# julienperriercornet/turbosqueeze

Measured on AMD Instinct MI355X. Metric: encode+decode GB/s on enwik9-shaped input (round trip of uncompressed bytes), higher is better.
Workload: dtype u8

## Files before the change

### include/turbosqueeze_amd.h

```cpp
#ifndef TURBOSQUEEZE_AMD_H
#define TURBOSQUEEZE_AMD_H

#include <stdbool.h>
#include <stddef.h>
#include <stdint.h>
#include <stdio.h>

#ifdef __cplusplus
extern "C" {
#endif

#ifndef TSQ_BLOCK_BITS
#define TSQ_BLOCK_BITS (22)
#define TSQ_BLOCK_SZ   (1 << TSQ_BLOCK_BITS)
#define TSQ_OUTPUT_SZ  ((1 << TSQ_BLOCK_BITS) + (1 << (TSQ_BLOCK_BITS - 2)))
#define TSQ_HASH_BITS  (17)
#define TSQ_HASH_SZ    ((1 << TSQ_HASH_BITS) * sizeof(uint16_t))
#define TSQ_HASH_MASK  ((1 << TSQ_HASH_BITS) - 1)
#endif

enum {
    TSQA_OK            = 0,
    TSQA_ERR_NO_DEVICE = 1,
    TSQA_ERR_HIP       = 2,
// ... 45 lines not shown
    uint32_t pad;
} tsqa_frame;

int tsqa_decode_blocks_async(tsqa_ctx *ctx, const void *d_streams, const tsqa_frame *d_frames, uint32_t n_blocks,
                             void *d_out, int32_t *d_status, void *hip_stream);

int tsqa_frames_to_host_async(tsqa_ctx *ctx, const void *d_slots, const uint32_t *sizes, const uint64_t *frame_at,
                              uint32_t n_blocks, uint32_t ext, void *host_container, void *hip_stream);
int tsqa_frames_from_host_async(tsqa_ctx *ctx, const void *host_container, const uint64_t *frame_at, const uint32_t *sizes,
                                uint32_t n_blocks, void *d_streams, void *hip_stream);

int tsqa_profile_enable(tsqa_ctx *ctx, int on);
int tsqa_profile_read(tsqa_ctx *ctx, double *encode_ms, uint32_t *encode_launches,
                      double *decode_ms, uint32_t *decode_launches);
int tsqa_profile_read_calls(tsqa_ctx *ctx, double *compress_ms, uint32_t *compress_calls,
                            double *decompress_ms, uint32_t *decompress_calls);

int tsqa_frame_offsets(const uint32_t *sizes, uint32_t n_blocks, uint64_t *frame_at, uint64_t *container_size);
int tsqa_walk_frames(const void *container, size_t size, uint32_t cap_blocks, uint64_t *frame_at, uint32_t *sizes, uint32_t *ext,
                     uint32_t *out_len, uint32_t *n_blocks, uint64_t *total);
int tsqa_sharded_place_async(tsqa_ctx *ctx, const void *d_slots, const uint32_t *all_sizes, uint32_t n_blocks, uint64_t n_total,
                             uint32_t rank, uint32_t world, uint32_t ext, void *host_container, size_t host_cap,
                             uint64_t *container_size, void *hip_stream);
int tsqa_sharded_fetch_decode_async(tsqa_ctx *ctx, const void *host_container, size_t container_size, uint32_t rank, uint32_t world,
                                    void *d_streams, size_t streams_cap, void *d_out, size_t out_cap, int32_t *d_status, uint64_t *total,
                                    void *hip_stream);
int tsqa_sharded_decode_again_async(tsqa_ctx *ctx, const void *d_streams, void *d_out, int32_t *d_status, void *hip_stream);

int tsqa_measure_copy(tsqa_ctx *ctx, size_t bytes, int reps, double *best_gbps, double *median_gbps);
const char *tsqa_copy_probe_shape(const tsqa_ctx *ctx);

void tsqa_set_kernel_variant(tsqa_ctx *ctx, int encode_variant, int decode_variant);
void tsqa_set_decode_wait_limit(tsqa_ctx *ctx, uint32_t polls);

typedef struct tsqa_index tsqa_index;
int      tsqa_index_create(tsqa_ctx *ctx, const void *d_container, size_t n, tsqa_index **out);
void     tsqa_index_destroy(tsqa_index *idx);
uint32_t tsqa_index_blocks(const tsqa_index *idx);
uint64_t tsqa_index_total(const tsqa_index *idx);

typedef struct tsqa_range { uint64_t offset, length, out_at; } tsqa_range;
typedef struct tsqa_range_item { uint32_t block, lo, hi, pad; uint64_t out_at; } tsqa_range_item;

int tsqa_plan_ranges(const uint64_t *out_start, uint32_t n_blocks, const tsqa_range *ranges, uint32_t n_ranges,
                     size_t out_cap, tsqa_range_item *items, uint32_t cap_items, uint32_t *n_items);

int tsqa_decompress_ranges_async(tsqa_ctx *ctx, const tsqa_index *idx, const tsqa_range *ranges, uint32_t n_ranges,
                                 void *d_out, size_t out_cap, int32_t *d_status, void *hip_stream);
int tsqa_decompress_ranges(tsqa_ctx *ctx, const tsqa_index *idx, const tsqa_range *ranges, uint32_t n_ranges,
                           void *d_out, size_t out_cap, void *hip_stream);

typedef struct tsqa_batch_item { uint64_t in_at, in_len, out_at, out_cap; } tsqa_batch_item;

int tsqa_plan_batch(const tsqa_batch_item *items, uint32_t n_items, size_t in_size, size_t out_size,
                    const uint32_t *n_blocks, uint64_t *first_block);

int tsqa_compress_batch_async(tsqa_ctx *ctx, const void *d_in, size_t in_size, const tsqa_batch_item *items, uint32_t n_items,
                              uint32_t ext, void *d_out, size_t out_size, uint64_t *d_sizes, int32_t *d_status, void *hip_stream);
int tsqa_compress_batch(tsqa_ctx *ctx, const void *d_in, size_t in_size, const tsqa_batch_item *items, uint32_t n_items,
                        uint32_t ext, void *d_out, size_t out_size, uint64_t *sizes, void *hip_stream);

int tsqa_decompress_batch_async(tsqa_ctx *ctx, const void *d_in, size_t in_size, const tsqa_batch_item *items,
                                const uint32_t *n_blocks, uint32_t n_items, void *d_out, size_t out_size,
                                uint64_t *d_sizes, int32_t *d_status, void *hip_stream);
int tsqa_decompress_batch(tsqa_ctx *ctx, const void *d_in, size_t in_size, const tsqa_batch_item *items, uint32_t n_items,
                          void *d_out, size_t out_size, uint64_t *sizes, int32_t *item_status, void *hip_stream);
// ... 121 lines not shown
```

### turbosqueeze_amd/api.py

```python
from __future__ import annotations

import ctypes as C
import os
import subprocess

HERE = os.path.dirname(os.path.abspath(__file__))
BLOCK_SZ = 1 << 22
OUTPUT_SZ = BLOCK_SZ + (BLOCK_SZ >> 2)

ERRORS = {1: "no usable gfx950 device", 2: "HIP runtime error", 3: "bad argument", 4: "malformed container",
          5: "malformed block stream", 6: "block expanded beyond TSQ_OUTPUT_SZ",
          7: "multi-workgroup decode stalled waiting for a sibling workgroup (the container may be fine: decode again with variant 4)"}


class TsqError(RuntimeError):
    def __init__(self, code: int, detail: str = ""):
        self.code = code
        super().__init__(f"turbosqueeze_amd error {code} ({ERRORS.get(code, '?')}) {detail}".strip())


def lib_path(ab=False) -> str:
    if isinstance(ab, str):
        return os.path.join(HERE, f"libturbosqueeze_amd_{ab}.so")
    return os.path.join(HERE, "libturbosqueeze_amd_ab.so" if ab else "libturbosqueeze_amd.so")
# ... 35 lines not shown
                          "(hipcc --offload-arch=gfx950); turbosqueeze_amd has no CPU fallback")
    L = C.CDLL(path)
    vp, u8pp, szp = C.c_void_p, C.POINTER(C.c_void_p), C.POINTER(C.c_size_t)
    L.tsqa_create.restype = C.c_int
    L.tsqa_create.argtypes = [C.c_int, C.POINTER(vp)]
    L.tsqa_destroy.restype = None
    L.tsqa_destroy.argtypes = [vp]
    L.tsqa_last_error.restype = C.c_char_p
    L.tsqa_last_error.argtypes = [vp]
    L.tsqa_device_id.restype = C.c_int
    L.tsqa_device_id.argtypes = [vp]
    L.tsqa_block_count.restype = C.c_size_t
    L.tsqa_block_count.argtypes = [C.c_size_t]
    L.tsqa_build_info.restype = C.c_char_p
    L.tsqa_build_info.argtypes = []
    L.tsqa_container_bound.restype = C.c_size_t
    L.tsqa_container_bound.argtypes = [C.c_size_t]
    L.tsqa_compress_device.restype = C.c_int
    L.tsqa_compress_device.argtypes = [vp, vp, C.c_size_t, vp, C.c_size_t, szp, C.c_uint32, vp]
    L.tsqa_compress_device_async.restype = C.c_int
    L.tsqa_compress_device_async.argtypes = [vp, vp, C.c_size_t, vp, C.c_size_t, vp, vp, C.c_uint32, vp]
    L.tsqa_decompress_device.restype = C.c_int
    L.tsqa_decompress_device.argtypes = [vp, vp, C.c_size_t, vp, C.c_size_t, szp, vp]
    L.tsqa_decompress_device_async.restype = C.c_int
    L.tsqa_decompress_device_async.argtypes = [vp, vp, C.c_size_t, C.c_uint32, vp, C.c_size_t, vp, vp, vp]
    L.tsqa_profile_enable.restype = C.c_int
    L.tsqa_profile_enable.argtypes = [vp, C.c_int]
    L.tsqa_profile_read.restype = C.c_int
    L.tsqa_profile_read.argtypes = [vp, C.POINTER(C.c_double), C.POINTER(C.c_uint32), C.POINTER(C.c_double), C.POINTER(C.c_uint32)]
    L.tsqa_set_kernel_variant.restype = None
    L.tsqa_set_kernel_variant.argtypes = [vp, C.c_int, C.c_int]
    L.tsqa_set_decode_wait_limit.restype = None
    L.tsqa_set_decode_wait_limit.argtypes = [vp, C.c_uint32]
    L.tsqAllocateContext.restype = vp
    L.tsqDeallocateContext.argtypes = [vp]
    L.tsqInit.argtypes = [vp]
    L.tsqEncode.restype = None
    L.tsqEncode.argtypes = [vp, vp, vp, C.POINTER(C.c_uint32), C.c_uint32, C.c_uint32]
    L.tsqDecode.restype = None
    L.tsqDecode.argtypes = [vp, vp, C.POINTER(C.c_uint32), C.c_uint32, C.c_uint32]
    L.tsqAllocateContextCompression_MT.restype = vp
    L.tsqAllocateContextCompression_MT.argtypes = [C.c_bool]
    L.tsqDeallocateContextCompression_MT.argtypes = [vp]
    L.tsqAllocateContextDecompression_MT.restype = vp
    L.tsqAllocateContextDecompression_MT.argtypes = [C.c_bool]
    L.tsqDeallocateContextDecompression_MT.argtypes = [vp]
    L.tsqCompress_MT.restype = C.c_bool
    L.tsqCompress_MT.argtypes = [vp, vp, C.c_size_t, C.c_bool, u8pp, szp, C.c_bool, C.c_bool, C.c_uint32]
    L.tsqDecompress_MT.restype = C.c_bool
    L.tsqDecompress_MT.argtypes = [vp, vp, C.c_size_t, C.c_bool, u8pp, szp, C.c_bool]
    L.tsqa_compress_async_cb.restype = C.c_uint32
    L.tsqa_compress_async_cb.argtypes = [vp, vp, C.c_size_t, C.c_bool, u8pp, szp, C.c_bool, C.c_bool, C.c_uint32, vp, vp, vp]
    L.tsqa_decompress_async_cb.restype = C.c_uint32
    L.tsqa_decompress_async_cb.argtypes = [vp, vp, C.c_size_t, C.c_bool, u8pp, szp, C.c_bool, vp, vp, vp]
    L.tsqa_profile_read_calls.restype = C.c_int
    L.tsqa_profile_read_calls.argtypes = [vp, C.POINTER(C.c_double), C.POINTER(C.c_uint32), C.POINTER(C.c_double), C.POINTER(C.c_uint32)]
    L.tsqa_encode_blocks_async.restype = C.c_int
    L.tsqa_encode_blocks_async.argtypes = [vp, vp, C.c_uint32, C.c_size_t, C.c_uint32, C.c_uint32, vp, vp, vp, vp]
    L.tsqa_decode_blocks_async.restype = C.c_int
    L.tsqa_decode_blocks_async.argtypes = [vp, vp, vp, C.c_uint32, vp, vp, vp]
    L.tsqa_frames_to_host_async.restype = C.c_int
    L.tsqa_frames_to_host_async.argtypes = [vp, vp, vp, vp, C.c_uint32, C.c_uint32, vp, vp]
    L.tsqa_frames_from_host_async.restype = C.c_int
    L.tsqa_frames_from_host_async.argtypes = [vp, vp, vp, vp, C.c_uint32, vp, vp]
    u32p, u64p = C.POINTER(C.c_uint32), C.POINTER(C.c_uint64)
    L.tsqa_frame_offsets.restype = C.c_int
# ... 457 lines not shown
        self.h = C.c_void_p()
        if device < 0:
            device = torch.cuda.current_device()
        rc = self.L.tsqa_create(device, C.byref(self.h))
        if rc:
            raise TsqError(rc)
        self.device = torch.device("cuda", device)
        self._size = torch.zeros(1, dtype=torch.int64, device=self.device)
        self._status = torch.zeros(1, dtype=torch.int32, device=self.device)

    def close(self):
        if self.h:
            self.L.tsqa_destroy(self.h)
            self.h = C.c_void_p()

    def __del__(self):
        try:
            self.close()
        except Exception:
            pass

    def _err(self, rc):
        return TsqError(rc, self.L.tsqa_last_error(self.h).decode())

    def last_error(self) -> str:
        return self.L.tsqa_last_error(self.h).decode()

    def set_variant(self, enc: int, dec: int) -> None:
        self.L.tsqa_set_kernel_variant(self.h, enc, dec)

    def set_decode_wait_limit(self, polls: int) -> None:
        self.L.tsqa_set_decode_wait_limit(self.h, polls)

    def profile(self, on: bool) -> None:
        self.L.tsqa_profile_enable(self.h, 1 if on else 0)

    def profile_read(self):
        em, dm, en, dn = C.c_double(0), C.c_double(0), C.c_uint32(0), C.c_uint32(0)
        self.L.tsqa_profile_read(self.h, C.byref(em), C.byref(en), C.byref(dm), C.byref(dn))
        return em.value, en.value, dm.value, dn.value

    def profile_read_calls(self):
        em, dm, en, dn = C.c_double(0), C.c_double(0), C.c_uint32(0), C.c_uint32(0)
        self.L.tsqa_profile_read_calls(self.h, C.byref(em), C.byref(en), C.byref(dm), C.byref(dn))
        return em.value, en.value, dm.value, dn.value

    def measure_copy(self, nbytes: int = 1 << 30, reps: int = 7):
        best, med = C.c_double(0), C.c_double(0)
        rc = self.L.tsqa_measure_copy(self.h, nbytes, reps, C.byref(best), C.byref(med))
        if rc:
            raise self._err(rc)
        return best.value, med.value

    def copy_probe_shape(self) -> str:
        return self.L.tsqa_copy_probe_shape(self.h).decode()

    def _stream(self):
        return C.c_void_p(self.torch.cuda.current_stream(self.device).cuda_stream)

    def encode_blocks_async(self, d_in, n_blocks: int, stride: int, last_len: int, ext: int, d_slots, d_sizes):
        rc = self.L.tsqa_encode_blocks_async(self.h, d_in.data_ptr(), n_blocks, stride, last_len, int(ext), d_slots.data_ptr(),
                                             d_sizes.data_ptr(), self._status.data_ptr(), self._stream())
        if rc:
            raise self._err(rc)

    def decode_blocks_async(self, d_streams, d_frames, n_blocks: int, d_out):
# ... 433 lines not shown
```

### turbosqueeze_amd/csrc/tsq_container.cuh

```cuda
#pragma once

#include "tsq_common.cuh"
#include "tsq_format.h"

namespace tsq {

__device__ __forceinline__ uint64_t group_scan_excl64(uint64_t v, uint64_t* wave_sum , uint64_t* total)
{
    const uint32_t lane = threadIdx.x & 63u, wid = threadIdx.x >> 6;
    const uint64_t incl = ((uint64_t)wave_scan_add((uint32_t)(v >> 24)) << 24) + wave_scan_add((uint32_t)v & 0xFFFFFFu);
    __syncthreads();
    if (lane == 63u) wave_sum[wid] = incl;
    __syncthreads();
    uint64_t before = 0, all = 0;
    for (uint32_t w = 0; w < 4u; ++w) { const uint64_t s = wave_sum[w]; if (w < wid) before += s; all += s; }
    *total = all;
    return before + incl - v;
}

__global__ __launch_bounds__(256) void pack_scan_kernel(const uint32_t* __restrict__ sizes, uint32_t n_blocks,
                                                        uint64_t n_total, uint32_t ext, uint8_t* __restrict__ container,
                                                        uint64_t out_cap, uint64_t* __restrict__ frame_at,
                                                        uint64_t* __restrict__ out_size, int32_t* __restrict__ status)
{
// ... 19 lines not shown

constexpr uint32_t kPackPiece = 32768;
__device__ __forceinline__ void pack_copy_piece(const uint8_t* src, uint32_t size, uint8_t* dst, uint32_t piece_at)
{
    const uint32_t head = (uint32_t)((16u - ((uintptr_t)dst & 15u)) & 15u);
    const uint32_t begin = piece_at + head;
    const uint32_t end_all = size;
    uint32_t end = begin + kPackPiece;
    if (end > end_all) end = end_all;
    if (piece_at == 0) for (uint32_t k = threadIdx.x; k < head && k < size; k += 256) dst[k] = src[k];
    if (begin >= end_all) return;
    const uint32_t words = (end - begin) >> 4;
    for (uint32_t w = threadIdx.x; w < words; w += 256) {
        uint4 v;
        __builtin_memcpy(&v, src + begin + (w << 4), 16);
        *reinterpret_cast<uint4*>(dst + begin + (w << 4)) = v;
    }
    if (end == end_all) for (uint32_t k = begin + (words << 4) + threadIdx.x; k < end_all; k += 256) dst[k] = src[k];
}

__global__ __launch_bounds__(256) void pack_copy_kernel(const uint8_t* __restrict__ slots, const uint32_t* __restrict__ sizes,
                                                        const uint64_t* __restrict__ frame_at, uint8_t* __restrict__ container,
                                                        const int32_t* __restrict__ status)
{
    const uint32_t b = blockIdx.y;
    const uint32_t size = sizes[b];
    const uint32_t piece_at = blockIdx.x * kPackPiece;
    if (piece_at >= size || *status != 0) return;
    pack_copy_piece(slots + (size_t)b * kSlotSize, size, container + frame_at[b] + 3, piece_at);
}

__global__ __launch_bounds__(64) void frame_walk_kernel(const uint8_t* __restrict__ container, uint64_t n, uint32_t n_blocks,
                                                        uint64_t out_cap, FrameInfo* __restrict__ frames,
                                                        uint64_t* __restrict__ out_size, int32_t* __restrict__ status)
{
    if (threadIdx.x != 0) return;
    uint32_t nb = 0;
    uint64_t total = 0;
    const bool ok = read_header(container, n, &nb, &total) == kHeaderOk && nb == n_blocks && total <= out_cap &&
                    walk_frames(container, n, nb, total, [&](uint32_t b, uint64_t, const FrameInfo& f) { frames[b] = f; return true; }) == kWalkOk;
    *out_size = ok ? total : 0;
    if (!ok) atomicMax(status, kErrFormat);
}

}
```

### turbosqueeze_amd/csrc/tsq_internal.h

```cpp
#pragma once

#include <hip/hip_runtime.h>
#include <stddef.h>
#include <stdint.h>
#include <utility>
#include <vector>

#include "../../include/turbosqueeze_amd.h"

namespace tsq { struct FrameInfo; struct BatchItem; struct EncBatchBlock; }

struct tsqa_ctx;

template <class T> struct tsqa_scratch {
    T* p = nullptr;
    size_t cap = 0;
    tsqa_scratch() = default;
    tsqa_scratch(const tsqa_scratch&) = delete;
    tsqa_scratch& operator=(const tsqa_scratch&) = delete;
    ~tsqa_scratch() { reset(); }
    operator T*() const { return p; }
    bool needs(size_t n) const { return n > cap; }
    void reset() { (void)hipFree(p); p = nullptr; cap = 0; }
    bool grow(tsqa_ctx* c, size_t n);
// ... 27 lines not shown

struct tsqa_ctx {
    int device = 0;
    int n_cus = 0;
    hipStream_t stream = nullptr;
    tsqa_scratch<uint8_t> slots;
    tsqa_scratch<uint32_t> sizes;
    tsqa_scratch<uint64_t> frame_at;
    tsqa_scratch<tsq::FrameInfo> frames;
    tsqa_scratch<uint32_t> block_owner;
    tsqa_scratch<uint16_t> tables;
    tsq::FrameInfo* host_frames = nullptr;
    size_t cap_host_frames = 0;
    std::vector<uint64_t> host_frame_src;
    hipEvent_t host_frames_copied = nullptr;
    bool host_frames_pending = false;
    uint32_t sharded_n_local = 0;
    const void* sharded_streams = nullptr;
    void* sharded_out = nullptr;
    void forget_sharded() { sharded_n_local = 0; sharded_streams = nullptr; sharded_out = nullptr; }
    tsqa_uploads range_up, batch_up;
    tsqa_scratch<int32_t> batch_status;
    tsqa_scratch<uint64_t> batch_at, batch_sizes, batch_offsets;
    tsqa_scratch<uint8_t> batch_heads;
    tsqa_scratch<tsq::BatchItem> batch_items;
    tsqa_scratch<uint32_t> batch_live;
    tsqa_scratch<tsq::EncBatchBlock> table_blocks;
    tsqa_scratch<uint32_t> table_launch_item;
    char probe_shape[160] = {0};
    tsqa_scratch<uint32_t> duo_ring;
    tsqa_scratch<uint32_t> duo_flags;
    tsqa_scratch<uint64_t> d_size;
    tsqa_scratch<int32_t> d_status;
    int enc_variant = 0, dec_variant = 0;
    uint32_t decode_wait_limit = 1u << 24;
    char err[256] = {0};
    static constexpr int kProfKinds = 4, kProfPairs = 256;
    bool profiling = false;
    std::vector<hipEvent_t> prof_pool;
    uint32_t prof_used[kProfKinds] = {0, 0, 0, 0};

    void set_error(const char* fmt, ...) __attribute__((format(printf, 2, 3)));
    void wait_for(hipStream_t s) { (void)hipStreamSynchronize(stream); if (s && s != stream) (void)hipStreamSynchronize(s); }
    int reserve(size_t n_blocks, bool want_tables, bool want_slots = true, bool all_streams = false, hipStream_t s = nullptr);
    int reserve_duo(size_t n_blocks, hipStream_t s = nullptr);
    int reserve_host_frames(size_t n);
    int reserve_batch(size_t n_items);
    int reserve_tables(size_t n_blocks, size_t n_launches);
    int launch_encode(const void* d_in, size_t n, size_t readable, uint32_t ext, int32_t* status, hipStream_t s);
    int launch_encode_to(const void* d_in, size_t n, size_t readable, size_t stride, uint32_t ext, uint8_t* slots_out,
                         uint32_t* sizes_out, int32_t* status, hipStream_t s);
    int launch_decode_frames(const void* d_streams, const tsq::FrameInfo* d_frames, uint32_t n_blocks, void* d_out, int32_t* status, hipStream_t s, int variant = -1);
    int decode_again(const void* d_streams, const tsq::FrameInfo* d_frames, uint32_t n_blocks, void* d_out, int32_t* status, hipStream_t s);
    int launch_pack(size_t n, uint32_t ext, void* d_out, size_t out_cap, uint64_t* d_out_size, int32_t* status, hipStream_t s);
};

template <class T> bool tsqa_scratch<T>::grow(tsqa_ctx* c, size_t n)
{
    if (!needs(n)) return true;
    reset();
    const hipError_t e = hipMalloc(&p, n * sizeof(T));
    if (e != hipSuccess) { p = nullptr; c->set_error("hipMalloc of %zu B failed: %s", n * sizeof(T), hipGetErrorString(e)); return false; }
    cap = n;
    return true;
}

// ... 15 lines not shown
```

### turbosqueeze_amd/csrc/tsq_runtime.hip

```cpp
#include "tsq_internal.h"

#include "tsq_batch.cuh"
#include "tsq_common.cuh"
#include "tsq_container.cuh"
#include "tsq_format.h"
#include "tsq_serial.cuh"
#include "tsq_split.cuh"
#include "tsq_index.cuh"
#include "tsq_launch.cuh"

#include <algorithm>
#include <cstdarg>
#include <cstdio>
#include <cstring>
#include <memory>
#include <new>

using namespace tsq;

#define TSQ_HIP(ctx, call)                                                                       \
    do {                                                                                         \
        hipError_t e_ = (call);                                                                  \
        if (e_ != hipSuccess) {                                                                  \
            (ctx)->set_error("%s failed: %s", #call, hipGetErrorString(e_));                     \
// ... 61 lines not shown
#endif
#ifdef TSQ_JITTER
           " TSQ_JITTER"
#endif
#if !TSQ_TIMING_ONLY_BUILD && !TSQ_INSTRUMENTED_BUILD
           " none"
#endif
           "]";
}

extern "C" int tsqa_create(int device, tsqa_ctx** out)
{
    if (!out) return TSQA_ERR_ARG;
    *out = nullptr;
    int count = 0;
    if (hipGetDeviceCount(&count) != hipSuccess || count <= 0) return TSQA_ERR_NO_DEVICE;
    if (device < 0) { if (hipGetDevice(&device) != hipSuccess) return TSQA_ERR_NO_DEVICE; }
    if (device >= count) return TSQA_ERR_ARG;
    hipDeviceProp_t prop;
    if (hipGetDeviceProperties(&prop, device) != hipSuccess) return TSQA_ERR_NO_DEVICE;
    if (strncmp(prop.gcnArchName, "gfx950", 6) != 0) {
        fprintf(stderr, "turbosqueeze_amd: device %d is %s; this library carries gfx950 code only\n", device, prop.gcnArchName);
        return TSQA_ERR_NO_DEVICE;
    }
    tsqa_ctx* c = new (std::nothrow) tsqa_ctx();
    if (!c) return TSQA_ERR_ARG;
    c->device = device;
    c->n_cus = prop.multiProcessorCount;
    if (const char* e = getenv("TSQ_AMD_DECODE_WAIT_LIMIT")) { const long v = atol(e); if (v > 0) c->decode_wait_limit = (uint32_t)v; }
    if (hipSetDevice(device) != hipSuccess || hipStreamCreateWithFlags(&c->stream, hipStreamNonBlocking) != hipSuccess) {
        delete c;
        return TSQA_ERR_HIP;
    }
    if (!c->d_size.grow(c, 1) || !c->d_status.grow(c, 1)) {
        tsqa_destroy(c);
        return TSQA_ERR_HIP;
    }
    *out = c;
    return TSQA_OK;
}

extern "C" void tsqa_destroy(tsqa_ctx* c)
{
    if (!c) return;
    (void)hipSetDevice(c->device);
    if (c->stream) { (void)hipStreamSynchronize(c->stream); (void)hipStreamDestroy(c->stream); }
    for (hipEvent_t e : c->prof_pool) if (e) (void)hipEventDestroy(e);
    if (c->host_frames) (void)hipHostFree(c->host_frames);
    if (c->host_frames_copied) (void)hipEventDestroy(c->host_frames_copied);
    c->range_up.destroy(); c->batch_up.destroy();
    delete c;
}

extern "C" const char* tsqa_last_error(const tsqa_ctx* c) { return c ? c->err : "null context"; }
extern "C" int tsqa_device_id(const tsqa_ctx* c) { return c ? c->device : -1; }
extern "C" void tsqa_set_kernel_variant(tsqa_ctx* c, int ev, int dv) { if (c) { c->enc_variant = ev; c->dec_variant = dv; } }
extern "C" void tsqa_set_decode_wait_limit(tsqa_ctx* c, uint32_t polls) { if (c) c->decode_wait_limit = polls ? polls : 1u; }

int tsqa_ctx::reserve(size_t n_blocks, bool want_tables, bool want_slots, bool all_streams, hipStream_t s)
{
    (void)hipSetDevice(device);
    const size_t nb = n_blocks, n_at = nb ? nb + 1 : 0;
    const size_t n_slots = want_slots && nb ? nb * (size_t)kSlotSize + 256 : 0, n_tables = want_tables ? nb * (size_t)kHashEntries : 0;
    const bool descriptors = sizes.needs(nb) || frame_at.needs(n_at) || frames.needs(nb) || block_owner.needs(nb);
    if (!descriptors && !slots.needs(n_slots) && !tables.needs(n_tables)) return TSQA_OK;
    if (all_streams) (void)hipDeviceSynchronize(); else wait_for(s);
    if (descriptors) forget_sharded();
    return sizes.grow(this, nb) && frame_at.grow(this, n_at) && frames.grow(this, nb) && block_owner.grow(this, nb) &&
           slots.grow(this, n_slots) && tables.grow(this, n_tables) ? TSQA_OK : TSQA_ERR_HIP;
}

int tsqa_ctx::reserve_duo(size_t n_blocks, hipStream_t s)
{
    (void)hipSetDevice(device);
    const size_t n_ring = n_blocks * (size_t)DuoCfg::SLOTS * DuoCfg::REC_WORDS, n_flags = n_blocks * (size_t)DuoCfg::FLAG_STRIDE;
    if (!duo_ring.needs(n_ring) && !duo_flags.needs(n_flags)) return TSQA_OK;
    wait_for(s);
    return duo_ring.grow(this, n_ring) && duo_flags.grow(this, n_flags) ? TSQA_OK : TSQA_ERR_HIP;
}

static size_t doubled(size_t from, size_t n)
{
    if (n == 0) return 0;
    while (from < n) from *= 2;
    return from;
}

int tsqa_ctx::reserve_host_frames(size_t n)
{
    (void)hipSetDevice(device);
    if (host_frames_pending) { (void)hipEventSynchronize(host_frames_copied); host_frames_pending = false; }
    if (!host_frames_copied) TSQ_HIP(this, hipEventCreateWithFlags(&host_frames_copied, hipEventDisableTiming));
    if (n > cap_host_frames) {
        if (host_frames) (void)hipHostFree(host_frames);
        host_frames = nullptr; cap_host_frames = 0;
        const size_t want = doubled(64, n);
        TSQ_HIP(this, hipHostMalloc(reinterpret_cast<void**>(&host_frames), want * sizeof(FrameInfo), hipHostMallocDefault));
        cap_host_frames = want;
    }
    host_frame_src.resize(cap_host_frames);
// ... 93 lines not shown
    }
    c->prof_used[kind] = 0;
    if (ms) *ms = sum;
    if (count) *count = n;
}

extern "C" int tsqa_profile_read(tsqa_ctx* c, double* enc_ms, uint32_t* enc_n, double* dec_ms, uint32_t* dec_n)
{
    if (!c) return TSQA_ERR_ARG;
    (void)hipSetDevice(c->device);
    if (c->prof_pool.empty()) { if (enc_ms) *enc_ms = 0; if (enc_n) *enc_n = 0; if (dec_ms) *dec_ms = 0; if (dec_n) *dec_n = 0; return TSQA_OK; }
    drain_events(c, 0, enc_ms, enc_n);
    drain_events(c, 1, dec_ms, dec_n);
    return TSQA_OK;
}

extern "C" int tsqa_profile_read_calls(tsqa_ctx* c, double* comp_ms, uint32_t* comp_n, double* decomp_ms, uint32_t* decomp_n)
{
    if (!c) return TSQA_ERR_ARG;
    (void)hipSetDevice(c->device);
    if (c->prof_pool.empty()) { if (comp_ms) *comp_ms = 0; if (comp_n) *comp_n = 0; if (decomp_ms) *decomp_ms = 0; if (decomp_n) *decomp_n = 0; return TSQA_OK; }
    drain_events(c, 2, comp_ms, comp_n);
    drain_events(c, 3, decomp_ms, decomp_n);
    return TSQA_OK;
}


int tsqa_ctx::launch_encode_to(const void* d_in, size_t n, size_t readable, size_t stride, uint32_t ext, uint8_t* slots_out,
                               uint32_t* sizes_out, int32_t* status, hipStream_t s)
{
    const uint32_t nb = (uint32_t)tsqa_block_count(n);
    int rc = reserve(nb, true, false, false, s);
    if (rc) return rc;
    ProfSpan span(this, 0, s);
    rc = launch_encode_kernels(this, static_cast<const uint8_t*>(d_in), n, readable, stride, ext, slots_out, sizes_out, status, s);
    if (rc) { span.cancel(); return rc; }
    span.end();
    TSQ_HIP(this, hipGetLastError());
    return TSQA_OK;
}

int tsqa_ctx::launch_encode(const void* d_in, size_t n, size_t readable, uint32_t ext, int32_t* status, hipStream_t s)
{
    int rc = reserve((uint32_t)tsqa_block_count(n), true, true, false, s);
    if (rc) return rc;
    return launch_encode_to(d_in, n, readable, kBlockSize, ext, slots, sizes, status, s);
}


static uint32_t pack_pieces(uint32_t max_stream = kSlotSize) { return (max_stream + kPackPiece - 1) / kPackPiece + 1; }

int tsqa_ctx::launch_pack(size_t n, uint32_t ext, void* d_out, size_t out_cap, uint64_t* d_out_size, int32_t* status, hipStream_t s)
{
    const uint32_t nb = (uint32_t)tsqa_block_count(n);
    hipLaunchKernelGGL(pack_scan_kernel, dim3(1), dim3(256), 0, s, sizes, nb, (uint64_t)n, ext,
                       static_cast<uint8_t*>(d_out), (uint64_t)out_cap, frame_at, d_out_size, status);
    hipLaunchKernelGGL(pack_copy_kernel, dim3(pack_pieces(), nb), dim3(256), 0, s, slots, sizes, frame_at,
                       static_cast<uint8_t*>(d_out), status);
    TSQ_HIP(this, hipGetLastError());
    return TSQA_OK;
}

int tsqa_ctx::launch_decode_frames(const void* d_streams, const FrameInfo* d_frames, uint32_t n_blocks, void* d_out, int32_t* status, hipStream_t s, int variant)
{
    ProfSpan span(this, 1, s);
    int rc = launch_decode_kernels(this, static_cast<const uint8_t*>(d_streams), d_frames, n_blocks, static_cast<uint8_t*>(d_out), status, s, variant);
    if (rc) { span.cancel(); return rc; }
    span.end();
    TSQ_HIP(this, hipGetLastError());
    return TSQA_OK;
}

int tsqa_ctx::decode_again(const void* d_streams, const FrameInfo* d_frames, uint32_t n_blocks, void* d_out, int32_t* status, hipStream_t s)
{
    TSQ_HIP(this, hipMemsetAsync(status, 0, sizeof(int32_t), s));
    return launch_decode_frames(d_streams, d_frames, n_blocks, d_out, status, s, 4);
}


extern "C" int tsqa_compress_device_async(tsqa_ctx* c, const void* d_in, size_t n, void* d_out, size_t out_cap,
                                          uint64_t* d_out_size, int32_t* d_status, uint32_t ext, void* hip_stream)
{
    if (!c) return TSQA_ERR_ARG;
    if (!d_in || !d_out || !d_out_size || !d_status || n == 0) { c->set_error("compress: null pointer or zero size"); return TSQA_ERR_ARG; }
    if (out_cap < 16 + 6 * tsqa_block_count(n)) { c->set_error("compress: output capacity too small"); return TSQA_ERR_ARG; }
    hipStream_t s = stream_of(c, hip_stream);
    (void)hipSetDevice(c->device);
    TSQ_HIP(c, hipMemsetAsync(d_status, 0, sizeof(int32_t), s));
    ProfSpan span(c, 2, s);
    int rc = c->launch_encode(d_in, n, n, ext, d_status, s);
    if (rc) { span.cancel(); return rc; }
    rc = c->launch_pack(n, ext, d_out, out_cap, d_out_size, d_status, s);
    span.end();
    return rc;
}

static int status_to_rc(tsqa_ctx* c, int32_t st, const char* what)
{
    if (st == 0) return TSQA_OK;
    c->set_error("%s: device reported status %d", what, st);
    return st;
}

static int read_status(tsqa_ctx* c, hipStream_t s, int32_t* st, size_t* out_size = nullptr)
{
    uint64_t sz = 0;
    if (out_size) TSQ_HIP(c, hipMemcpyAsync(&sz, c->d_size, sizeof(sz), hipMemcpyDeviceToHost, s));
    TSQ_HIP(c, hipMemcpyAsync(st, c->d_status, sizeof(int32_t), hipMemcpyDeviceToHost, s));
    TSQ_HIP(c, hipStreamSynchronize(s));
    if (out_size) *out_size = (size_t)sz;
    return TSQA_OK;
}
static int finish_sync(tsqa_ctx* c, hipStream_t s, const char* what, size_t* out_size = nullptr)
{
    int32_t st = 0;
    if (int rc = read_status(c, s, &st, out_size)) return rc;
    return status_to_rc(c, st, what);
}

extern "C" int tsqa_compress_device(tsqa_ctx* c, const void* d_in, size_t n, void* d_out, size_t out_cap,
                                    size_t* out_size, uint32_t ext, void* hip_stream)
{
    if (!c || !out_size) return TSQA_ERR_ARG;
    hipStream_t s = stream_of(c, hip_stream);
    int rc = tsqa_compress_device_async(c, d_in, n, d_out, out_cap, c->d_size, c->d_status, ext, s);
    if (rc) return rc;
    return finish_sync(c, s, "compress", out_size);
}

static int decompress_device_async_impl(tsqa_ctx* c, const void* d_in, size_t n, uint32_t n_blocks, void* d_out,
                                        size_t out_cap, uint64_t* d_out_size, int32_t* d_status, void* hip_stream, int variant,
                                        bool sized = false, const uint32_t* d_block_sizes = nullptr)
{
    if (!c) return TSQA_ERR_ARG;
    if (!d_in || !d_out || !d_out_size || !d_status || n < 16 || n_blocks == 0 || (sized && !d_block_sizes)) { c->set_error("decompress: bad argument"); return TSQA_ERR_ARG; }
    hipStream_t s = stream_of(c, hip_stream);
    (void)hipSetDevice(c->device);
    int rc = c->reserve(n_blocks, false, false, false, s);
    if (rc) return rc;
    c->forget_sharded();
    TSQ_HIP(c, hipMemsetAsync(d_status, 0, sizeof(int32_t), s));
    ProfSpan span(c, 3, s);
    if (sized)
        hipLaunchKernelGGL(frame_walk_sized_kernel, dim3(1), dim3(256), 0, s, static_cast<const uint8_t*>(d_in), (uint64_t)n, n_blocks,
                           d_block_sizes, (uint64_t)out_cap, c->frames, d_out_size, d_status);
    else
        hipLaunchKernelGGL(frame_walk_kernel, dim3(1), dim3(64), 0, s, static_cast<const uint8_t*>(d_in), (uint64_t)n, n_blocks,
                           (uint64_t)out_cap, c->frames, d_out_size, d_status);
    rc = c->launch_decode_frames(d_in, c->frames, n_blocks, d_out, d_status, s, variant);
    span.end();
    return rc;
}

extern "C" int tsqa_decompress_device_async(tsqa_ctx* c, const void* d_in, size_t n, uint32_t n_blocks, void* d_out,
                                            size_t out_cap, uint64_t* d_out_size, int32_t* d_status, void* hip_stream)
{
    return decompress_device_async_impl(c, d_in, n, n_blocks, d_out, out_cap, d_out_size, d_status, hip_stream, -1);
}

extern "C" int tsqa_decompress_device_sized_async(tsqa_ctx* c, const void* d_in, size_t n, uint32_t n_blocks, const uint32_t* d_block_sizes,
                                                  void* d_out, size_t out_cap, uint64_t* d_out_size, int32_t* d_status, void* hip_stream)
{
    return decompress_device_async_impl(c, d_in, n, n_blocks, d_out, out_cap, d_out_size, d_status, hip_stream, -1, true, d_block_sizes);
}


extern "C" int tsqa_encode_blocks_async(tsqa_ctx* c, const void* d_in, uint32_t n_blocks, size_t stride, uint32_t last_len,
                                        uint32_t ext, void* d_slots, uint32_t* d_sizes, int32_t* d_status, void* hip_stream)
{
    if (!c) return TSQA_ERR_ARG;
    if (!d_in || !d_slots || !d_sizes || !d_status || n_blocks == 0 || last_len == 0 || last_len > kBlockSize || stride < kBlockSize) {
        c->set_error("encode_blocks: bad argument");
        return TSQA_ERR_ARG;
    }
    hipStream_t s = stream_of(c, hip_stream);
    (void)hipSetDevice(c->device);
    TSQ_HIP(c, hipMemsetAsync(d_status, 0, sizeof(int32_t), s));
    const size_t n = (size_t)(n_blocks - 1) * kBlockSize + last_len;
    const size_t tail = stride > kBlockSize ? (stride - kBlockSize < 128 ? stride - kBlockSize : 128) : 0;
    const size_t readable = (size_t)(n_blocks - 1) * stride + last_len + tail;
    return c->launch_encode_to(d_in, n, readable, stride, ext, static_cast<uint8_t*>(d_slots), d_sizes, d_status, s);
// ... 203 lines not shown
    IndexPtr idx(new (std::nothrow) tsqa_index());
    try {
        if (!idx) throw std::bad_alloc();
        idx->device = c->device; idx->container = static_cast<const uint8_t*>(d_container); idx->n = n; idx->n_blocks = nb; idx->total = total;
        if (host_copy) idx->host_frames.resize(nb);
        if (one_item) {
            idx->out_start.resize((size_t)nb + 1);
            idx->item_first = {0ull, (uint64_t)nb};
            idx->item_status = {TSQA_OK};
        }
    } catch (...) { c->set_error("%s: out of host memory", who); idx.reset(); }
    return idx;
}

extern "C" int tsqa_index_create(tsqa_ctx* c, const void* d_container, size_t n, tsqa_index** out)
{
    if (!out) return TSQA_ERR_ARG;
    *out = nullptr;
    if (!c) return TSQA_ERR_ARG;
    if (!d_container) { c->set_error("index_create: null container"); return TSQA_ERR_ARG; }
    if (n < kHeaderSize) { c->set_error("index_create: a container of %zu B has no header", n); return TSQA_ERR_FORMAT; }
    (void)hipSetDevice(c->device);
    hipStream_t s = c->stream;
    uint8_t head[kHeaderSize];
    TSQ_HIP(c, hipMemcpyAsync(head, d_container, kHeaderSize, hipMemcpyDeviceToHost, s));
    TSQ_HIP(c, hipStreamSynchronize(s));
    uint32_t nb; uint64_t total;
    if (read_header(head, n, &nb, &total) != kHeaderOk) { c->set_error("index_create: bad header"); return TSQA_ERR_FORMAT; }
    IndexPtr idx = index_begin(c, "index_create", d_container, n, nb, total, true, true);
    if (!idx) return TSQA_ERR_ARG;
    int32_t st = 0;
    TSQ_HIP(c, hipMalloc(&idx->frames, (size_t)nb * sizeof(FrameInfo)));
    TSQ_HIP(c, hipMemsetAsync(c->d_status, 0, sizeof(int32_t), s));
    hipLaunchKernelGGL(frame_walk_kernel, dim3(1), dim3(64), 0, s, idx->container, (uint64_t)n, nb, total, idx->frames, c->d_size, c->d_status);
    TSQ_HIP(c, hipGetLastError());
    TSQ_HIP(c, hipMemcpyAsync(&st, c->d_status, sizeof(st), hipMemcpyDeviceToHost, s));
    TSQ_HIP(c, hipMemcpyAsync(idx->host_frames.data(), idx->frames, (size_t)nb * sizeof(FrameInfo), hipMemcpyDeviceToHost, s));
    TSQ_HIP(c, hipStreamSynchronize(s));
    if (st != 0) { c->set_error("index_create: malformed container (status %d)", st); return TSQA_ERR_FORMAT; }
    for (uint32_t b = 0; b < nb; ++b) idx->out_start[b] = idx->host_frames[b].out_at;
    idx->out_start[nb] = total;
    *out = idx.release();
    return TSQA_OK;
}

extern "C" int tsqa_index_create_sized_async(tsqa_ctx* c, const void* d_container, size_t n, uint64_t n_total, uint32_t block_len,
                                             const uint32_t* d_block_sizes, tsqa_index** out, void* hip_stream)
{
    if (!out) return TSQA_ERR_ARG;
    *out = nullptr;
    if (!c) return TSQA_ERR_ARG;
    if (!d_container || !d_block_sizes) { c->set_error("index_create_sized: null pointer"); return TSQA_ERR_ARG; }
    uint32_t nb = 0;
    size_t bound = 0;
    if (n_total > (uint64_t)SIZE_MAX || tsqa_plan_split((size_t)n_total, block_len, &nb, &bound)) {
        c->set_error("index_create_sized: no data, a block_len that is no power of two from 2^12 to 2^22, or more than 2^32 - 1 blocks");
        return TSQA_ERR_ARG;
    }
    if (n < kHeaderSize + (uint64_t)kMinFrameSize * nb) { c->set_error("index_create_sized: %zu B cannot hold %u frames", n, nb); return TSQA_ERR_ARG; }
    hipStream_t s = stream_of(c, hip_stream);
    (void)hipSetDevice(c->device);
    IndexPtr idx = index_begin(c, "index_create_sized", d_container, n, nb, n_total, true, false);
    if (!idx) return TSQA_ERR_ARG;
    for (uint32_t b = 0; b < nb; ++b) idx->out_start[b] = (uint64_t)b * block_len;
    idx->out_start[nb] = n_total;
    const uint32_t n_groups = (uint32_t)(((uint64_t)nb + kIndexGroup - 1u) / kIndexGroup);
    const size_t frames_bytes = (size_t)nb * sizeof(FrameInfo), bytes = frames_bytes + ((size_t)n_groups + 1u) * sizeof(uint64_t);
// ... 288 lines not shown
        if (mode == kPlanPacked) { blocks += nb; continue; }
        if (x.out_cap > out_size || x.out_at > out_size - x.out_cap) { *why = "an output range ends past out_size"; return TSQA_ERR_ARG; }
        if (mode == kPlanCompress && x.out_cap < kHeaderSize + kMinFrameSize * nb) { *why = "an output range holds less than 16 + 6 bytes per block"; return TSQA_ERR_ARG; }
        if ((mode == kPlanDecompress || mode == kPlanRangesOnly) && x.in_len < kHeaderSize) { *why = "an input range is shorter than a header"; return TSQA_ERR_ARG; }
        if (mode == kPlanDecompress && (nb == 0 || nb > (x.in_len - kHeaderSize) / kMinFrameSize)) { *why = "a block count that the container cannot hold"; return TSQA_ERR_ARG; }
        if (x.out_cap) dst.emplace_back(x.out_at, x.out_cap);
        blocks += nb;
    }
    if (destinations_overlap(dst)) { *why = "two output ranges overlap"; return TSQA_ERR_ARG; }
    if (blocks > 0xFFFFFFFFull) { *why = "more than 2^32 - 1 blocks"; return TSQA_ERR_ARG; }
    if (mode == kPlanRangesOnly) return TSQA_OK;
    uint64_t at = 0;
    for (uint32_t i = 0; i < n_items; ++i) { first_block[i] = at; at += blocks_of(i); }
    first_block[n_items] = at;
    return TSQA_OK;
}

extern "C" int tsqa_plan_batch(const tsqa_batch_item* items, uint32_t n_items, size_t in_size, size_t out_size, const uint32_t* n_blocks,
                               uint64_t* first_block)
{
    const char* why;
    if (!first_block) return TSQA_ERR_ARG;
    return plan_batch(items, n_items, in_size, out_size, n_blocks, first_block, &why, n_blocks ? kPlanDecompress : kPlanCompress);
}

static uint32_t batch_budget(const tsqa_ctx* c) { return 2u * (uint32_t)c->n_cus; }

template <class Scan>
static int batch_route_enqueue(tsqa_ctx* c, const uint8_t* in, const EncBatchBlock* blocks, uint64_t n_blocks, uint32_t ext, uint32_t pieces,
                               uint8_t* out, const uint32_t* live, int32_t* d_status, hipStream_t s, Scan scan)
{
    const uint32_t budget = batch_budget(c);
    uint32_t launch = 0;
    for (uint64_t b0 = 0; b0 < n_blocks; b0 += budget, ++launch) {
        const uint32_t nb = (uint32_t)(n_blocks - b0 < budget ? n_blocks - b0 : budget), first = live ? (uint32_t)b0 : 0u;
        ProfSpan span(c, 0, s);
        const int rc = launch_batch_encode_kernels(c, in, blocks + b0, nb, ext, c->slots, c->sizes, d_status, s, first, live);
        if (rc) { span.cancel(); return rc; }
        span.end();
        scan(b0, nb, launch);
        hipLaunchKernelGGL(batch_pack_copy_kernel, dim3(pieces, nb), dim3(256), 0, s, c->slots, c->sizes, c->frame_at, out, first, live);
    }
    return TSQA_OK;
}

static int compress_batch_enqueue(tsqa_ctx* c, const void* d_in, const tsqa_batch_item* items, uint32_t n_items, const std::vector<uint64_t>& first,
                                  uint32_t ext, void* d_out, size_t out_size, uint32_t align, uint64_t* d_offsets, uint64_t* d_sizes,
                                  int32_t* d_status, hipStream_t s)
{
    static_assert(sizeof(tsqa_batch_item) == 32 && sizeof(BatchItem) == 48 && sizeof(EncBatchBlock) == 24, "descriptor layouts");
    (void)hipSetDevice(c->device);
    const uint64_t n_blocks = first[n_items];
    const uint32_t budget = batch_budget(c);
    const size_t item_bytes = (size_t)n_items * sizeof(BatchItem), bytes = item_bytes + n_blocks * sizeof(EncBatchBlock);
    tsqa_uploads::Slot up;
    if (int rc = c->batch_up.acquire(c, bytes, &up)) return rc;
    if (int rc = c->reserve(n_blocks < budget ? n_blocks : budget, true, true, true)) return rc;
    if (int rc = c->reserve_batch(n_items)) return rc;
    BatchItem* const hi = up.host<BatchItem>();
    EncBatchBlock* const hb = up.host<EncBatchBlock>(item_bytes);
    for (uint32_t i = 0; i < n_items; ++i) {
        const tsqa_batch_item& x = items[i];
        const uint32_t nb = (uint32_t)(first[i + 1] - first[i]);
        hi[i] = align ? BatchItem{x.in_at, x.in_len, 0, 0, first[i], nb, 0u} : BatchItem{x.in_at, x.in_len, x.out_at, x.out_cap, first[i], nb, 0u};
        for (uint32_t j = 0; j < nb; ++j) {
            const uint64_t b = first[i] + j, off = (uint64_t)j * kBlockSize, left = x.in_len - off;
// ... 716 lines not shown
```

### turbosqueeze_amd/csrc/tsq_split.cuh

```cuda
#pragma once

#include "tsq_batch.cuh"
#include "tsq_common.cuh"
#include "tsq_container.cuh"
#include "tsq_format.h"

namespace tsq {

__global__ __launch_bounds__(256) void split_blocks_kernel(uint64_t n, uint32_t block_len, uint32_t n_blocks, uint32_t budget,
                                                           EncBatchBlock* __restrict__ blocks)
{
    const uint64_t b = (uint64_t)blockIdx.x * 256u + threadIdx.x;
    if (b >= n_blocks) return;
    const uint64_t at = b * block_len, left = n - at;
    blocks[b] = EncBatchBlock{at, left, left < block_len ? (uint32_t)left : block_len, (uint32_t)(b % budget)};
}

__global__ __launch_bounds__(256) void split_pack_scan_kernel(const uint32_t* __restrict__ sizes, uint32_t b0, uint32_t nb, uint32_t n_blocks,
                                                              uint64_t n_total, uint32_t ext, uint32_t max_stream, uint8_t* __restrict__ out,
                                                              uint64_t out_cap,
                                                              uint64_t* __restrict__ run_at, uint64_t* __restrict__ frame_at,
                                                              uint64_t* __restrict__ out_size, uint32_t* __restrict__ block_sizes,
                                                              int32_t* __restrict__ status)
{
// ... 2 lines not shown
    uint64_t base = b0 == 0u ? (uint64_t)kHeaderSize : *run_at;
    if (b0 == 0u && t == 0u && kHeaderSize <= out_cap) write_header(out, n_blocks, n_total);
    for (uint32_t k0 = 0; k0 < nb; k0 += 256u) {
        const uint32_t k = k0 + t;
        const bool valid = k < nb;
        const uint32_t sz = valid ? sizes[k] : 0u;
        uint64_t sum;
        const uint64_t at = base + group_scan_excl64(valid ? kFrameWordSize + (uint64_t)sz : 0ull, wave_sum, &sum);
        base += sum;
        if (valid) {
            const bool fits = at + kFrameWordSize + sz <= out_cap;
            if (fits) write_frame(out + at, sz, ext);
            frame_at[k] = fits ? at : kNoFrame;
            if (block_sizes) block_sizes[b0 + k] = sz;
            if (sz > max_stream) atomicMax(status, kErrOverflow);
        }
    }
    if (t != 0u) return;
    *run_at = base;
    if (b0 + nb == n_blocks) {
        *out_size = base;
        if (base > out_cap) atomicMax(status, kErrOverflow);
    }
}

__device__ __forceinline__ bool sized_frame_ok(const uint8_t* container, uint64_t n, uint64_t at, bool s_ok, uint32_t s, FrameInfo* f)
{
    return s_ok && at + kMinFrameSize <= n && read_frame(container + at, at, n, f) && f->stream_len == s;
}

__global__ __launch_bounds__(256) void frame_walk_sized_kernel(const uint8_t* __restrict__ container, uint64_t n, uint32_t n_blocks,
                                                               const uint32_t* __restrict__ table, uint64_t out_cap,
                                                               FrameInfo* __restrict__ frames, uint64_t* __restrict__ out_size,
                                                               int32_t* __restrict__ status)
{
    __shared__ uint64_t wave_sum[4];
    const uint32_t t = threadIdx.x;
    uint32_t nb = 0;
    uint64_t total = 0;
    if (!(read_header(container, n, &nb, &total) == kHeaderOk && nb == n_blocks && total <= out_cap)) {
        if (t == 0u) { *out_size = 0; atomicMax(status, kErrFormat); }
        return;
    }
    uint64_t at_base = kHeaderSize, oat_base = 0;
    bool bad = false;
    for (uint64_t b0 = 0; b0 < nb; b0 += 256u) {
        const uint64_t b = b0 + t;
        const bool valid = b < nb;
        const uint32_t s = valid ? table[b] : 0u;
        const bool s_ok = valid && stream_len_ok(s);
        uint64_t sum;
        const uint64_t at = at_base + group_scan_excl64(s_ok ? kFrameWordSize + (uint64_t)s : 0ull, wave_sum, &sum);
        at_base += sum;
        FrameInfo f{0, 0, 0, 0, 0, 0};
        const bool f_ok = sized_frame_ok(container, n, at, s_ok, s, &f);
        const uint32_t out_len = f_ok ? f.out_len : 0u;
        const uint64_t oat = oat_base + group_scan_excl64(out_len, wave_sum, &sum);
        oat_base += sum;
        const bool fits = f_ok && oat + out_len <= total;
        if (fits) { f.stream_at = at + kFrameWordSize; f.out_at = oat; frames[b] = f; }
        if (valid && !fits) bad = true;
    }
    const bool refused = __syncthreads_or(bad ? 1 : 0) != 0 || oat_base != total;
    if (t != 0u) return;
    *out_size = refused ? 0ull : total;
    if (refused) atomicMax(status, kErrFormat);
}

}
```

Measured before the change: 22.78.

## Reuse encoder block sizes as a hint for parallel frame walk on decode

When decoding a container that this context just produced on the same stream, the block sizes left over from encode are reused. They let the 256-thread sized frame walk (a parallel prefix scan) run in place of the serial single-thread walk. The serial walk kernel is still launched but exits at once unless the hinted walk flags a mismatch, in which case it falls back. This adds a kernel launch and state kept across calls, and relies on the kept sizes still matching the container.

```diff
diff --git a/include/turbosqueeze_amd.h b/include/turbosqueeze_amd.h
--- a/include/turbosqueeze_amd.h
+++ b/include/turbosqueeze_amd.h
@@ -101,6 +101,7 @@
 
 void tsqa_set_kernel_variant(tsqa_ctx *ctx, int encode_variant, int decode_variant);
 void tsqa_set_decode_wait_limit(tsqa_ctx *ctx, uint32_t polls);
+int tsqa_last_walk_kind(tsqa_ctx *ctx, int *kind);
 
 typedef struct tsqa_index tsqa_index;
 int      tsqa_index_create(tsqa_ctx *ctx, const void *d_container, size_t n, tsqa_index **out);
diff --git a/turbosqueeze_amd/api.py b/turbosqueeze_amd/api.py
--- a/turbosqueeze_amd/api.py
+++ b/turbosqueeze_amd/api.py
@@ -91,6 +91,8 @@
     L.tsqa_set_kernel_variant.argtypes = [vp, C.c_int, C.c_int]
     L.tsqa_set_decode_wait_limit.restype = None
     L.tsqa_set_decode_wait_limit.argtypes = [vp, C.c_uint32]
+    L.tsqa_last_walk_kind.restype = C.c_int
+    L.tsqa_last_walk_kind.argtypes = [vp, C.POINTER(C.c_int)]
     L.tsqAllocateContext.restype = vp
     L.tsqDeallocateContext.argtypes = [vp]
     L.tsqInit.argtypes = [vp]
@@ -614,6 +616,13 @@
     def set_decode_wait_limit(self, polls: int) -> None:
         self.L.tsqa_set_decode_wait_limit(self.h, polls)
 
+    def last_walk_kind(self) -> int:
+        k = C.c_int(0)
+        rc = self.L.tsqa_last_walk_kind(self.h, C.byref(k))
+        if rc:
+            raise self._err(rc)
+        return k.value
+
     def profile(self, on: bool) -> None:
         self.L.tsqa_profile_enable(self.h, 1 if on else 0)
 
diff --git a/turbosqueeze_amd/csrc/tsq_container.cuh b/turbosqueeze_amd/csrc/tsq_container.cuh
--- a/turbosqueeze_amd/csrc/tsq_container.cuh
+++ b/turbosqueeze_amd/csrc/tsq_container.cuh
@@ -75,9 +75,10 @@
 
 __global__ __launch_bounds__(64) void frame_walk_kernel(const uint8_t* __restrict__ container, uint64_t n, uint32_t n_blocks,
                                                         uint64_t out_cap, FrameInfo* __restrict__ frames,
-                                                        uint64_t* __restrict__ out_size, int32_t* __restrict__ status)
+                                                        uint64_t* __restrict__ out_size, int32_t* __restrict__ status,
+                                                        const uint32_t* __restrict__ hint_missed)
 {
-    if (threadIdx.x != 0) return;
+    if (threadIdx.x != 0 || (hint_missed && *hint_missed == 0u)) return;
     uint32_t nb = 0;
     uint64_t total = 0;
     const bool ok = read_header(container, n, &nb, &total) == kHeaderOk && nb == n_blocks && total <= out_cap &&
diff --git a/turbosqueeze_amd/csrc/tsq_internal.h b/turbosqueeze_amd/csrc/tsq_internal.h
--- a/turbosqueeze_amd/csrc/tsq_internal.h
+++ b/turbosqueeze_amd/csrc/tsq_internal.h
@@ -83,6 +83,14 @@
     tsqa_scratch<uint32_t> duo_flags;
     tsqa_scratch<uint64_t> d_size;
     tsqa_scratch<int32_t> d_status;
+    const void* kept_container = nullptr;
+    size_t kept_bytes = 0;
+    uint32_t kept_blocks = 0;
+    hipStream_t kept_stream = nullptr;
+    void forget_kept() { kept_container = nullptr; kept_bytes = 0; kept_blocks = 0; kept_stream = nullptr; }
+    tsqa_scratch<uint32_t> walk_missed;
+    bool walk_hinted = false;
+    hipStream_t walk_stream = nullptr;
     int enc_variant = 0, dec_variant = 0;
     uint32_t decode_wait_limit = 1u << 24;
     char err[256] = {0};
diff --git a/turbosqueeze_amd/csrc/tsq_runtime.hip b/turbosqueeze_amd/csrc/tsq_runtime.hip
--- a/turbosqueeze_amd/csrc/tsq_runtime.hip
+++ b/turbosqueeze_amd/csrc/tsq_runtime.hip
@@ -117,7 +117,7 @@
         delete c;
         return TSQA_ERR_HIP;
     }
-    if (!c->d_size.grow(c, 1) || !c->d_status.grow(c, 1)) {
+    if (!c->d_size.grow(c, 1) || !c->d_status.grow(c, 1) || !c->walk_missed.grow(c, 1)) {
         tsqa_destroy(c);
         return TSQA_ERR_HIP;
     }
@@ -150,7 +150,7 @@
     const bool descriptors = sizes.needs(nb) || frame_at.needs(n_at) || frames.needs(nb) || block_owner.needs(nb);
     if (!descriptors && !slots.needs(n_slots) && !tables.needs(n_tables)) return TSQA_OK;
     if (all_streams) (void)hipDeviceSynchronize(); else wait_for(s);
-    if (descriptors) forget_sharded();
+    if (descriptors) { forget_sharded(); forget_kept(); }
     return sizes.grow(this, nb) && frame_at.grow(this, n_at) && frames.grow(this, nb) && block_owner.grow(this, nb) &&
            slots.grow(this, n_slots) && tables.grow(this, n_tables) ? TSQA_OK : TSQA_ERR_HIP;
 }
@@ -310,6 +310,7 @@
     const uint32_t nb = (uint32_t)tsqa_block_count(n);
     int rc = reserve(nb, true, false, false, s);
     if (rc) return rc;
+    if (sizes_out == sizes) forget_kept();
     ProfSpan span(this, 0, s);
     rc = launch_encode_kernels(this, static_cast<const uint8_t*>(d_in), n, readable, stride, ext, slots_out, sizes_out, status, s);
     if (rc) { span.cancel(); return rc; }
@@ -370,7 +371,22 @@
     if (rc) { span.cancel(); return rc; }
     rc = c->launch_pack(n, ext, d_out, out_cap, d_out_size, d_status, s);
     span.end();
-    return rc;
+    if (rc) return rc;
+    c->kept_container = d_out; c->kept_bytes = out_cap; c->kept_blocks = (uint32_t)tsqa_block_count(n); c->kept_stream = s;
+    return TSQA_OK;
+}
+
+extern "C" int tsqa_last_walk_kind(tsqa_ctx* c, int* kind)
+{
+    if (!c || !kind) return TSQA_ERR_ARG;
+    (void)hipSetDevice(c->device);
+    *kind = 0;
+    if (!c->walk_hinted) return TSQA_OK;
+    uint32_t missed = 0;
+    TSQ_HIP(c, hipMemcpyAsync(&missed, c->walk_missed, sizeof(missed), hipMemcpyDeviceToHost, c->walk_stream));
+    TSQ_HIP(c, hipStreamSynchronize(c->walk_stream));
+    *kind = missed ? 2 : 1;
+    return TSQA_OK;
 }
 
 static int status_to_rc(tsqa_ctx* c, int32_t st, const char* what)
@@ -418,13 +434,20 @@
     if (rc) return rc;
     c->forget_sharded();
     TSQ_HIP(c, hipMemsetAsync(d_status, 0, sizeof(int32_t), s));
+    const bool hinted = !sized && c->kept_container == d_in && c->kept_stream == s && c->kept_blocks == n_blocks && n <= c->kept_bytes;
+    c->walk_hinted = hinted; c->walk_stream = s;
     ProfSpan span(c, 3, s);
     if (sized)
         hipLaunchKernelGGL(frame_walk_sized_kernel, dim3(1), dim3(256), 0, s, static_cast<const uint8_t*>(d_in), (uint64_t)n, n_blocks,
-                           d_block_sizes, (uint64_t)out_cap, c->frames, d_out_size, d_status);
-    else
+                           d_block_sizes, (uint64_t)out_cap, c->frames, d_out_size, d_status, static_cast<uint32_t*>(nullptr));
+    else {
+        uint32_t* hint_missed = hinted ? c->walk_missed.p : nullptr;
+        if (hinted)
+            hipLaunchKernelGGL(frame_walk_sized_kernel, dim3(1), dim3(256), 0, s, static_cast<const uint8_t*>(d_in), (uint64_t)n, n_blocks,
+                               static_cast<const uint32_t*>(c->sizes), (uint64_t)out_cap, c->frames, d_out_size, d_status, hint_missed);
         hipLaunchKernelGGL(frame_walk_kernel, dim3(1), dim3(64), 0, s, static_cast<const uint8_t*>(d_in), (uint64_t)n, n_blocks,
-                           (uint64_t)out_cap, c->frames, d_out_size, d_status);
+                           (uint64_t)out_cap, c->frames, d_out_size, d_status, static_cast<const uint32_t*>(hint_missed));
+    }
     rc = c->launch_decode_frames(d_in, c->frames, n_blocks, d_out, d_status, s, variant);
     span.end();
     return rc;
@@ -694,7 +717,7 @@
     int32_t st = 0;
     TSQ_HIP(c, hipMalloc(&idx->frames, (size_t)nb * sizeof(FrameInfo)));
     TSQ_HIP(c, hipMemsetAsync(c->d_status, 0, sizeof(int32_t), s));
-    hipLaunchKernelGGL(frame_walk_kernel, dim3(1), dim3(64), 0, s, idx->container, (uint64_t)n, nb, total, idx->frames, c->d_size, c->d_status);
+    hipLaunchKernelGGL(frame_walk_kernel, dim3(1), dim3(64), 0, s, idx->container, (uint64_t)n, nb, total, idx->frames, c->d_size, c->d_status, static_cast<const uint32_t*>(nullptr));
     TSQ_HIP(c, hipGetLastError());
     TSQ_HIP(c, hipMemcpyAsync(&st, c->d_status, sizeof(st), hipMemcpyDeviceToHost, s));
     TSQ_HIP(c, hipMemcpyAsync(idx->host_frames.data(), idx->frames, (size_t)nb * sizeof(FrameInfo), hipMemcpyDeviceToHost, s));
@@ -1049,6 +1072,7 @@
 {
     const uint32_t budget = batch_budget(c);
     uint32_t launch = 0;
+    c->forget_kept();
     for (uint64_t b0 = 0; b0 < n_blocks; b0 += budget, ++launch) {
         const uint32_t nb = (uint32_t)(n_blocks - b0 < budget ? n_blocks - b0 : budget), first = live ? (uint32_t)b0 : 0u;
         ProfSpan span(c, 0, s);
diff --git a/turbosqueeze_amd/csrc/tsq_split.cuh b/turbosqueeze_amd/csrc/tsq_split.cuh
--- a/turbosqueeze_amd/csrc/tsq_split.cuh
+++ b/turbosqueeze_amd/csrc/tsq_split.cuh
@@ -58,14 +58,14 @@
 __global__ __launch_bounds__(256) void frame_walk_sized_kernel(const uint8_t* __restrict__ container, uint64_t n, uint32_t n_blocks,
                                                                const uint32_t* __restrict__ table, uint64_t out_cap,
                                                                FrameInfo* __restrict__ frames, uint64_t* __restrict__ out_size,
-                                                               int32_t* __restrict__ status)
+                                                               int32_t* __restrict__ status, uint32_t* __restrict__ hint_missed)
 {
     __shared__ uint64_t wave_sum[4];
     const uint32_t t = threadIdx.x;
     uint32_t nb = 0;
     uint64_t total = 0;
     if (!(read_header(container, n, &nb, &total) == kHeaderOk && nb == n_blocks && total <= out_cap)) {
-        if (t == 0u) { *out_size = 0; atomicMax(status, kErrFormat); }
+        if (t == 0u) { if (hint_missed) *hint_missed = 1u; else { *out_size = 0; atomicMax(status, kErrFormat); } }
         return;
     }
     uint64_t at_base = kHeaderSize, oat_base = 0;
@@ -89,6 +89,7 @@
     }
     const bool refused = __syncthreads_or(bad ? 1 : 0) != 0 || oat_base != total;
     if (t != 0u) return;
+    if (hint_missed) { *hint_missed = refused ? 1u : 0u; if (refused) return; }
     *out_size = refused ? 0ull : total;
     if (refused) atomicMax(status, kErrFormat);
 }
```

After: 22.81 (median of 6 runs). About the same (+0.2%).
